# Ren91/gelly-streaming

Hardware: AMD Instinct MI355X
Metric: edges/sec per tumbling slice (reduceOnEdges, window triangles) at 1/2/4/8 GPUs (higher is better)
Workload: dtype int64

## Files before the change

gelly-streaming_amd/csrc/gs_bucket.hip:

```cpp
#include <algorithm>

#include "gs_ops.hpp"
#include <atomic>
#include <chrono>
#ifndef GS_DOM_ACCUM
#define GS_DOM_ACCUM 1
#endif

#include "gs_bucket.hpp"

namespace gs {

#ifndef GS_BK_ITEM_LOG
#define GS_BK_ITEM_LOG 17
#endif
#ifndef GS_BK_UNROLL
#define GS_BK_UNROLL 8
#endif
constexpr uint32_t BK_ITEM = 1u << GS_BK_ITEM_LOG;

namespace {

constexpr gs_status GS_RETRY_WIDE = -100;

struct BkMeta {
  static constexpr size_t HIST = 0, DBASE = HIST + BK_MAXB, BSTART = DBASE + 512, BCOUNT = BSTART + BK_MAXB + 4,
                          BITEMS = BCOUNT + BK_MAXB, BSLAB = BITEMS + BK_MAXB, MLIST = BSLAB + BK_MAXB,
                          MAXIT = MLIST + BK_MAXB,
                          TOTAL = MAXIT + 4;
};

struct BkGeom {
  int64_t base = 0;
  uint32_t nb = 1;
  int passes = 0, w = 0;
};

int64_t key_min(const uint64_t* h) { return (int64_t)(~h[0] ^ (1ull << 63)); }
int64_t key_max(const uint64_t* h) { return (int64_t)(h[1] ^ (1ull << 63)); }

int64_t predict_base(int64_t kmin, int64_t kmax, int S) {
  return (kmin >= 0 && ((uint64_t)kmax >> S) < (uint64_t)BK_MAXB) ? 0 : kmin;
}

template <int DIR>
// ... 74 lines not shown
uint32_t item_records(gs_ctx* c, uint64_t R) {
  const uint64_t per = R / (GS_BK_ITEMS_PER_CU * (uint64_t)std::max(1, c->n_cu));
  return (uint32_t)std::max<uint64_t>(BK_ITEM, std::min<uint64_t>(per, 1u << 20));
}

gs_status ensure_cu(gs_ctx* c) {
  if (!c->n_cu) {
    int cu = 0;
    GS_HIP(hipDeviceGetAttribute(&cu, hipDeviceAttributeMultiprocessorCount, c->device));
    c->n_cu = std::max(1, cu);
  }
  return GS_OK;
}

template <class P>
gs_status launch_plan(gs_ctx* c, uint64_t R, uint32_t nb, int passes, int w, uint32_t item_recs,
                      const uint32_t* cursor = nullptr, uint32_t* counts_out = nullptr,
                      unsigned long long* occupied = nullptr) {
  char* sm = c->small.as<char>();
  uint32_t* meta = c->bk_meta.as<uint32_t>();
  const uint64_t max_items = R / item_recs + nb + 1;
  const uint64_t max_slabs = 2 * (R / item_recs) + 2;
  GS_TRY(ensure(c, c->bk_items, max_items * sizeof(BkItem)));
  GS_TRY(ensure(c, c->bk_slabs, max_slabs * sizeof(typename P::Lds)));
  uint32_t* ns = (uint32_t*)(sm + SM_BK_N);
  BkPlanOut po{meta + BkMeta::DBASE, meta + BkMeta::BSTART, meta + BkMeta::BCOUNT, meta + BkMeta::BITEMS,
               meta + BkMeta::BSLAB, meta + BkMeta::MLIST, c->bk_items.as<BkItem>(), ns + 0, ns + 1,
               cursor, counts_out, occupied, ns + 2, meta + BkMeta::MAXIT};
  hipLaunchKernelGGL(k_bk_plan, dim3(1), dim3(BK_PLAN_BLOCK), 0, c->stream, meta + BkMeta::HIST, nb, passes, w,
                     item_recs, po);
  return hip_check(c, hipGetLastError(), "k_bk_plan");
}

template <class P, class Src>
gs_status bucket_accumulate(gs_ctx* c, Src rs, uint64_t R, uint32_t nb, int64_t base, typename P::Out o, int ev0,
                           const uint32_t* seg_cur = nullptr) {
  char* sm = c->small.as<char>();
  uint32_t* meta = c->bk_meta.as<uint32_t>();
  uint32_t* ns = (uint32_t*)(sm + SM_BK_N);
  const auto* mm = (const unsigned long long*)(sm + SM_BK_MM);
  BkStage st{c->keysA.as<uint32_t>(), c->valsA.p,
             (std::is_same_v<P, BkDeg> || std::is_same_v<P, BkDeg32>) ? c->aux.as<int64_t>() : nullptr};
  auto* slabs = c->bk_slabs.as<typename P::Lds>();
  const bool dom = GS_DOM_ACCUM && ev0 == 2 && c->timing == GS_TIMING_DOMINANT;
  launch_dominant(c, dom ? c->pass_ev[7] : nullptr, dom ? c->pass_ev[ev0 + 1] : nullptr, k_bk_accum<P, Src, GS_BK_UNROLL>,
                  dim3(c->n_cu * GS_BK_ACC_PER_CU), dim3(BK_ACC_BLOCK), rs, (const BkItem*)c->bk_items.as<BkItem>(),
                  (const uint32_t*)(ns + 0), (const uint32_t*)(meta + BkMeta::BSTART), ns + 2, slabs, st,
                  meta + BkMeta::BCOUNT, mm, seg_cur);
  GS_HIP(hipGetLastError());
  stage_event(c, c->pass_ev[ev0 + 1]);
  const unsigned mgrid = (unsigned)std::max<uint64_t>(1, std::min<uint64_t>({(uint64_t)nb, R / BK_ITEM + 1, 64}));
  const unsigned fgrid = (unsigned)std::max<uint64_t>(1, std::min<uint64_t>({(uint64_t)nb, R / BK_ITEM + 1, (uint64_t)c->n_cu}));
  hipLaunchKernelGGL((k_bk_merge_groups<P>), dim3(2048), dim3(BK_MS_BLOCK), 0, c->stream, meta + BkMeta::MLIST, ns + 1,
                     meta + BkMeta::BITEMS, meta + BkMeta::BSLAB, slabs, mm, (const uint32_t*)(meta + BkMeta::MAXIT));
  hipLaunchKernelGGL((k_bk_merge_slices<P>), dim3(mgrid, BK_MS_SLICES), dim3(BK_MS_BLOCK), 0, c->stream,
                     meta + BkMeta::MLIST, ns + 1, meta + BkMeta::BITEMS, meta + BkMeta::BSLAB, slabs, mm);
  hipLaunchKernelGGL((k_bk_merge<P>), dim3(fgrid), dim3(BK_ACC_BLOCK), 0, c->stream, meta + BkMeta::MLIST, ns + 1,
                     meta + BkMeta::BITEMS, meta + BkMeta::BSLAB, meta + BkMeta::BSTART, slabs, st,
                     meta + BkMeta::BCOUNT, mm);
  GS_HIP(hipGetLastError());
  stage_event(c, c->pass_ev[ev0 + 2]);
  if (c->oe.nparts) {
    const OwnerEmit& e = c->oe;
    hipLaunchKernelGGL(k_bk_owner_count, dim3(nb, BK_OE_SLICES), dim3(256), 0, c->stream, (const uint32_t*)(meta + BkMeta::BSTART),
                       (const uint32_t*)(meta + BkMeta::BCOUNT), nb, (const uint32_t*)st.k, base, e.nparts, e.cnt, e.wide,
                       mm, (const uint32_t*)(sm + SM_TIMEOUT), (const unsigned long long*)(sm + SM_BK_ESC),
                       (unsigned long long*)(sm + SM_BK_X));
    hipLaunchKernelGGL(k_owner_scan, dim3(1), dim3(1024), 0, c->stream, e.cnt, nb * BK_OE_SLICES * e.nparts,
                       nb * BK_OE_SLICES, e.nparts, e.totals,
                       (unsigned long long*)(sm + SM_BK_MM + 24));
    hipLaunchKernelGGL((k_bk_owner_emit<P>), dim3(nb, BK_OE_SLICES), dim3(256), 0, c->stream, (const uint32_t*)(meta + BkMeta::BSTART),
                       (const uint32_t*)(meta + BkMeta::BCOUNT), nb, st, base, o, e.nparts, (const uint32_t*)e.cnt, e.rows,
                       (const unsigned long long*)e.wide, e.vw, e.mw, mm);
    hipLaunchKernelGGL(k_send_rows, dim3(1), dim3(64), 0, c->stream, (const unsigned long long*)e.totals, e.wide,
// ... 169 lines not shown
        SpSlots slots{};
        const uint32_t xmask = c->sp_slot == 0 ? 7u : 0u;
        if (!xmask) {
          for (uint32_t x = 1; x <= SP_NSEG; ++x) slots.pre[x] = (uint32_t)R;
        } else {
          const uint64_t tr = (DIR == DIR_ALL ? 2 : 1) * SPTE, nfull = n / SPTE, per = (nfull + 7) / 8;
          uint64_t acc = 0;
          for (uint32_t x = 0; x < SP_NSEG; ++x) {
            slots.pre[x] = (uint32_t)acc;
            const uint64_t lo = std::min<uint64_t>(nfull, SP_NSEG == 1 ? 0 : x * per);
            const uint64_t hi = SP_NSEG == 1 ? nfull : std::min<uint64_t>(nfull, (x + 1) * per);
            acc += (hi - lo) * tr + (x == 0 ? R - nfull * tr : 0);
          }
          slots.pre[SP_NSEG] = (uint32_t)acc;
        }
        hipLaunchKernelGGL(k_sp_regions, dim3(1), dim3(BK_PLAN_BLOCK), 0, c->stream, (const uint32_t*)sp.tot.as<uint32_t>(),
                           nb, sp.R, R, meta + BkMeta::BSTART, c->sp_cur.as<uint32_t>(), slots, mm,
                           (unsigned long long*)(sm + SM_BK_ESC));
        if constexpr (P::REL) GS_HIP(hipMemsetAsync(rel_bad, 0, 4, c->stream));
        stage_event(c, c->ev[1]);
        stage_event(c, c->pass_ev[0]);
        stage_event(c, c->pass_ev[1]);
        using Load = typename P::Load;
        const BaseSrc<Load, DIR, P::PAY> ls{src, dst, (const Load*)val, base};
        uint32_t* cur = c->sp_cur.as<uint32_t>();
        hipEvent_t e0 = c->pass_ev[1], e1 = c->pass_ev[2];
        uint32_t* kp = c->keysB.as<uint32_t>();
        auto* esc = (unsigned long long*)(sm + SM_BK_ESC);
        const uint32_t trash = (uint32_t)cap;
        if constexpr (CAN_PACK && ITEMS == PK_ITEMS) {
          if (pack && nb <= 1024)
            launch_dominant(c, e0, e1, k_sp_scatter_pack<Load, DIR, 1024>, dim3(spk_grid<DIR>(n)), dim3(SPK_BLOCK), ls, n,
                            S, nb, cur, kp, vpart, trash, mm, esc, xmask);
// ... 2 lines not shown
                            n, S, nb, cur, kp, vpart, trash, mm, esc, xmask);
        }
        if constexpr (ITEMS == DP_ITEMS) {
          if (!pack) {
            if (nb <= 1024)
              launch_dominant(c, e0, e1, k_sp_scatter<Load, DIR, P::PAY, Raw, P::REL, 1024>, dim3(spu_grid<DIR>(n)),
                              dim3(SPU_BLOCK), ls, n, S, nb, cur, k16, vpart, trash, rel_bad, mm, xmask);
            else
              launch_dominant(c, e0, e1, k_sp_scatter<Load, DIR, P::PAY, Raw, P::REL, BK_MAXB>, dim3(spu_grid<DIR>(n)),
                              dim3(SPU_BLOCK), ls, n, S, nb, cur, k16, vpart, trash, rel_bad, mm, xmask);
          }
        }
        GS_HIP(hipGetLastError());
        stage_event(c, c->pass_ev[2]);
        stage_event(c, c->ev[2]);
        GS_TRY(launch_plan<P>(c, cap, nb, 0, 0, item_recs, cur, sp.tot.as<uint32_t>(), mm));
        part = true;
        if (pack) GS_TRY((bucket_accumulate<P>(c, PackSrc<Raw>{c->keysB.as<uint32_t>(), vpart}, cap, nb, base, o, 2, cur)));
        else GS_TRY((bucket_accumulate<P>(c, PartSrc<Raw>{k16, vpart}, cap, nb, base, o, 2, cur)));
        if (defer) return GS_PENDING_LOCAL;
        GS_TRY(bucket_wait(c));
        if (!c->host_small[2]) {
          kmin = (int64_t)((uint64_t)base + (c->host_small[0] << S));
          kmax = (int64_t)((uint64_t)base + (c->host_small[1] << S) + ((1ull << S) - 1));
          break;
        }
        sp.skip = 8;
        spec = false;
        spec_missed = true;
        continue;
      }
    }
    GS_TRY((launch_dp_hist<DIR, ITEMS>(c, src, dst, n, nt, base, S, nb)));
    GS_HIP(hipMemsetAsync(sm + SM_BK_ESC, 0, 8, c->stream));
// ... 76 lines not shown
  const uint64_t esc = pack ? c->host_small[7] : 0;
  const uint32_t key_bits = nb <= 1 ? (uint32_t)S : (uint32_t)(S + 32 - __builtin_clz(nb - 1));
  const size_t pb = pack ? 2 : (P::HAS_V ? sizeof(Raw) : 0);
  bucket_times(c, 2, part ? 1 : 0, 5, key_bits, R, *U, pb, n_items);
  c->times.key_bytes = 2;
  c->times.escapes = esc;
  c->times.packed = pack ? 1u : 0u;
  c->times.speculative = spec ? 1u : spec_missed ? 2u : 0u;
  if constexpr (SPEC_OK) {
    if (part) {
      sp.ok = true;
      sp.base = base;
      sp.S = S;
      sp.dir = DIR;
      sp.R = R;
    }
  }
  return GS_OK;
}

template <class P, int DIR>
gs_status bucket_direct(gs_ctx* c, const int64_t* src, const int64_t* dst, const void* val, uint64_t n,
                        typename P::Out o, uint64_t* U) {
  constexpr bool CAN_PACK = P::PAY == PAY_VAL && !P::REL && std::is_integral_v<typename P::A>;
  if constexpr (CAN_PACK) {
    if (c->bk_wide_vals[c->sp_slot] <= 0 && !(c->flags & GS_FLAG_NO_PACK))
      return bucket_direct_t<P, DIR, PK_ITEMS>(c, src, dst, val, n, o, U, true);
  }
  return bucket_direct_t<P, DIR, DP_ITEMS>(c, src, dst, val, n, o, U, false);
}
// ... 144 lines not shown
```

gelly-streaming_amd/csrc/gs_bucket.hpp:

```cpp
#pragma once
#include <limits>
#include <type_traits>

#include "gs_radix.hpp"
#include "gs_rbk.hpp"

namespace gs {

constexpr int BK_MAXB = 2048;
constexpr int BK_INFO_BLOCK = 512;
#ifndef GS_BK_ACC_BLOCK
#define GS_BK_ACC_BLOCK 1024
#endif
#ifndef GS_BK_ACC_PER_CU
#define GS_BK_ACC_PER_CU 1
#endif
#ifndef GS_BK_PREFETCH
#define GS_BK_PREFETCH 0
#endif
#ifndef GS_BK_FUSED_RESET
#define GS_BK_FUSED_RESET 1
#endif
#ifndef GS_BK_S8
#define GS_BK_S8 14
#endif
constexpr int BK_ACC_BLOCK = GS_BK_ACC_BLOCK;
constexpr int BK_NW = BK_ACC_BLOCK / WAVE;
constexpr int BK_PLAN_BLOCK = 1024;

struct BkItem {
  uint32_t bucket, begin, end, slab;
};

struct BkStage {
  uint32_t* k;
  void* a;
  int64_t* b;
};

struct BkPlanOut {
  uint32_t* digit_base;
  uint32_t* bucket_start;
  uint32_t* bucket_count;
  uint32_t* b_items;
  uint32_t* b_slab;
  uint32_t* mlist;
  BkItem* items;
  uint32_t* n_items;
  uint32_t* n_multi;
  const uint32_t* cursor = nullptr;
  uint32_t* counts_out = nullptr;
  unsigned long long* occupied = nullptr;
  uint32_t* claim = nullptr;
  uint32_t* max_items = nullptr;
};

#ifndef GS_SP_XCD
#define GS_SP_XCD 1
#endif
constexpr uint32_t SP_NSEG = GS_SP_XCD ? 8 : 1;
#ifndef GS_SP_MATCH
#define GS_SP_MATCH 1
#endif
constexpr uint32_t SP_PAD = 1024;
constexpr uint32_t SP_PADSEG = SP_PAD / SP_NSEG;
static_assert(SP_PADSEG % 4 == 0, "segment starts stay 4-aligned");
constexpr uint32_t SP_END_OFF = SP_NSEG * BK_MAXB;
constexpr uint32_t SP_LO_OFF = 2 * SP_NSEG * BK_MAXB;
constexpr uint32_t SP_CUR_WORDS = 3 * SP_NSEG * BK_MAXB;
// ... 419 lines not shown
#pragma unroll
  for (int i = 0; i < NW; ++i) {
    const uint32_t v = s_w[i];
    off += i < w ? v : 0u;
    tot += v;
  }
  __syncthreads();
  total = tot;
  return off + inc - x;
}

#ifndef GS_BK_LPT
#define GS_BK_LPT 1
#endif
constexpr int BK_LPT_CLASSES = 64;
static __global__ __launch_bounds__(BK_PLAN_BLOCK) void k_bk_plan(const uint32_t* __restrict__ hist, uint32_t nb,
                                                                  int passes, int w, uint32_t item_recs,
                                                                  BkPlanOut o) {
  __shared__ uint32_t s_dh[2][256];
  __shared__ uint32_t s_w[BK_PLAN_BLOCK / WAVE];
  __shared__ uint32_t s_maxit;
  const int tid = threadIdx.x;
  for (int i = tid; i < 2 * 256; i += BK_PLAN_BLOCK) (&s_dh[0][0])[i] = 0;
  if (tid == 0) s_maxit = 0;
  if (tid == 0 && o.claim) *o.claim = 0;
  __syncthreads();
  const uint32_t b0 = 2 * tid, b1 = 2 * tid + 1;
  const bool spec = o.cursor != nullptr;
  auto count = [&](uint32_t b) -> uint32_t {
    if (b >= nb) return 0u;
    if (!spec) return hist[b];
    uint32_t n = 0;
    for (uint32_t x = 0; x < SP_NSEG; ++x) n += min(o.cursor[x * BK_MAXB + b], sp_hi(o.cursor, x, b)) - sp_lo(o.cursor, x, b);
    return n;
  };
  const uint32_t c0 = count(b0), c1 = count(b1);
  const uint32_t dmask = (1u << w) - 1;
  for (int p = 0; p < passes; ++p) {
    if (c0) atomicAdd(&s_dh[p][(b0 >> (p * w)) & dmask], c0);
// ... 22 lines not shown
    o.counts_out[b0] = c0;
    o.counts_out[b1] = c1;
  }
  if (!spec) {
    if (b0 < nb) o.bucket_start[b0] = start0;
    if (b1 < nb) o.bucket_start[b1] = start0 + c0;
    if (tid == 0) o.bucket_start[nb] = total;
  }
  if (tid < passes) {
    uint32_t run = 0;
    for (uint32_t d = 0; d <= dmask; ++d) {
      o.digit_base[tid * 256 + d] = run;
      run += s_dh[tid][d];
    }
  }
  auto nitems = [&](uint32_t c) { return c == 0 ? 0u : (c + item_recs - 1) / item_recs; };
  const uint32_t i0 = nitems(c0), i1 = nitems(c1);
  const uint32_t m0 = i0 > 1 ? i0 : 0u, m1 = i1 > 1 ? i1 : 0u;
  uint32_t n_items, n_slabs, n_multi;
  const uint32_t first0 = bk_block_scan(i0 + i1, s_w, n_items);
  const uint32_t slab0 = bk_block_scan(m0 + m1, s_w, n_slabs);
  const uint32_t mb0 = bk_block_scan((m0 ? 1u : 0u) + (m1 ? 1u : 0u), s_w, n_multi);
#if GS_BK_LPT
  __shared__ uint32_t s_cls[BK_LPT_CLASSES];
  for (int i = tid; i < BK_LPT_CLASSES; i += BK_PLAN_BLOCK) s_cls[i] = 0;
  __syncthreads();
  auto size_class = [&](uint32_t n) -> uint32_t {
    return BK_LPT_CLASSES - 1 - min<uint32_t>(BK_LPT_CLASSES - 1, (uint32_t)((uint64_t)n * BK_LPT_CLASSES / (item_recs + 1)));
  };
  auto count_items = [&](uint32_t b, uint32_t c, uint32_t ni) {
    if (b >= nb || !ni) return;
    if (ni > 1) atomicAdd(&s_cls[size_class(item_recs)], ni - 1);
    atomicAdd(&s_cls[size_class(c - (ni - 1) * item_recs)], 1u);
  };
  count_items(b0, c0, i0);
  count_items(b1, c1, i1);
  __syncthreads();
  static_assert(BK_LPT_CLASSES == WAVE, "one wave scans the classes");
  if (tid < WAVE) {
    const uint32_t x = s_cls[tid];
    s_cls[tid] = wave_inclusive_sum(x) - x;
  }
  __syncthreads();
#endif
  auto emit_bucket = [&](uint32_t b, uint32_t c, uint32_t ni, uint32_t first, uint32_t slab, uint32_t mb) {
    if (b >= nb) return;
    o.bucket_count[b] = 0;
    o.b_items[b] = ni;
    o.b_slab[b] = slab;
    if (ni > 1) o.mlist[mb] = b;
    if (!ni) return;
#if GS_BK_LPT
    const uint32_t fpos = ni > 1 ? atomicAdd(&s_cls[size_class(item_recs)], ni - 1) : 0u;
    const uint32_t lpos = atomicAdd(&s_cls[size_class(c - (ni - 1) * item_recs)], 1u);
#endif
    for (uint32_t k = 0; k < ni; ++k) {
      BkItem it;
      it.bucket = b;
      it.begin = k * item_recs;
      it.end = min(c, (k + 1) * item_recs);
      it.slab = ni > 1 ? slab + k : ~0u;
#if GS_BK_LPT
      o.items[k + 1 < ni ? fpos + k : lpos] = it;
#else
      o.items[first + k] = it;
#endif
    }
  };
  emit_bucket(b0, c0, i0, first0, slab0, mb0);
  emit_bucket(b1, c1, i1, first0 + i0, slab0 + m0, mb0 + (m0 ? 1u : 0u));
  if (o.max_items) {
    if (i0 > 1 || i1 > 1) atomicMax(&s_maxit, max(i0, i1));
    __syncthreads();
  }
  if (tid == 0) {
    if (o.max_items) *o.max_items = s_maxit;
    *o.n_items = n_items;
    *o.n_multi = n_multi;
  }
}

#ifndef GS_DP_ITEMS
#define GS_DP_ITEMS 10
#endif
#ifndef GS_DP_XCD
#define GS_DP_XCD 1
#endif
#ifndef GS_DP_VDIRECT
#define GS_DP_VDIRECT 0
#endif
constexpr int DP_BLOCK = 1024;
constexpr int DP_ITEMS = GS_DP_ITEMS;
constexpr uint32_t DP_TILE = DP_BLOCK * DP_ITEMS;
constexpr uint32_t DP_CHUNK = 64;
// ... 383 lines not shown
    for (int u = 0; u < ITEMS; ++u) put((uint32_t)u * DP_BLOCK + tid);
  } else {
    for (uint32_t j = tid; j < nrec; j += DP_BLOCK) put(j);
  }
#pragma unroll
  for (int o = 32; o > 0; o >>= 1) esc += __shfl_xor(esc, o, WAVE);
  if ((tid & 63) == 0 && esc) atomicAdd(n_esc, (unsigned long long)esc);
}


static __global__ __launch_bounds__(BK_PLAN_BLOCK) void k_sp_regions(const uint32_t* __restrict__ prev, uint32_t nb,
                                                                     uint64_t r_prev, uint64_t r_now,
                                                                     uint32_t* __restrict__ bucket_start,
                                                                     uint32_t* __restrict__ cursor, SpSlots slots,
                                                                     unsigned long long* __restrict__ mm,
                                                                     unsigned long long* __restrict__ n_esc) {
  __shared__ uint32_t s_w[BK_PLAN_BLOCK / WAVE];
  __shared__ uint32_t s_frac[SP_NSEG + 1];
  const int tid = threadIdx.x;
  const uint32_t b0 = 2 * tid, b1 = 2 * tid + 1;
  if (tid <= (int)SP_NSEG) {
    const uint32_t all = slots.pre[SP_NSEG];
    const uint64_t f = all ? ((uint64_t)slots.pre[tid] << 32) / all : 0;
    s_frac[tid] = (uint32_t)min(f, (uint64_t)0xFFFFFFFFu);
  }
  auto cap = [&](uint32_t b) -> uint32_t {
    if (b >= nb) return 0u;
    const uint64_t t = (uint64_t)prev[b] * r_now / (r_prev ? r_prev : 1);
    return (uint32_t)((t + (t >> 4) + 3) & ~3ull) + SP_PAD;
  };
  const uint32_t c0 = cap(b0), c1 = cap(b1);
// ... 6 lines not shown
    const uint32_t h0 = sp_seg_start(s0, s0 + c0, x + 1, s_frac), h1 = sp_seg_start(s0 + c0, s0 + c0 + c1, x + 1, s_frac);
    if (b0 < nb) {
      cursor[x * BK_MAXB + b0] = l0;
      cursor[SP_LO_OFF + x * BK_MAXB + b0] = l0;
      cursor[SP_END_OFF + x * BK_MAXB + b0] = h0;
    }
    if (b1 < nb) {
      cursor[x * BK_MAXB + b1] = l1;
      cursor[SP_LO_OFF + x * BK_MAXB + b1] = l1;
      cursor[SP_END_OFF + x * BK_MAXB + b1] = h1;
    }
    l0 = h0;
    l1 = h1;
  }
  if (tid == 0) bucket_start[nb] = total;
  if (tid < 4) mm[tid] = 0;
  if (tid == 4) *n_esc = 0;
}

__host__ __device__ inline uint64_t sp_capacity(uint64_t r_now, uint32_t nb) {
  return r_now + (r_now >> 4) + (uint64_t)nb * (SP_PAD + 4);
}

#ifndef GS_SPK_BLOCK
#define GS_SPK_BLOCK 512
#endif
#ifndef GS_SPK_ITEMS
#define GS_SPK_ITEMS 16
#endif
#ifndef GS_SPK_NT
#define GS_SPK_NT 0
#endif
// ... 460 lines not shown
    const uint64_t m = ballot(p);
    if (p) {
      const uint32_t pos = stage_at + off + mbcnt(m);
      st.k[pos] = cbase | e;
      P::stage(st, pos, s, e);
    }
    off += (uint32_t)__popcll(m);
  }
  if constexpr (RESET) {
    static_assert(PER % 32 == 0, "a wave's entries are whole presence words");
    P::init_range(s, e0, e0 + PER, lane);
  }
  if (tid == 0) bucket_count[bucket] = tot;
}

#ifdef GS_BK_TRACE
constexpr uint32_t BK_TRACE_MAX = 16384;
__device__ uint64_t g_bk_trace[BK_TRACE_MAX][4];
#endif
template <class P, class Src, int UNROLL>
__global__ __launch_bounds__(BK_ACC_BLOCK) void k_bk_accum(Src src, const BkItem* __restrict__ items,
                                                           const uint32_t* __restrict__ n_items_p,
                                                           const uint32_t* __restrict__ bucket_start,
                                                           uint32_t* __restrict__ ctr,
                                                           typename P::Lds* __restrict__ slabs, BkStage st,
                                                           uint32_t* __restrict__ bucket_count,
                                                           const unsigned long long* __restrict__ mm,
                                                           const uint32_t* __restrict__ seg_cur) {
  __shared__ typename P::Lds s;
  __shared__ uint32_t s_item[2], s_b0[2];
  __shared__ BkItem s_m[2];
  __shared__ uint32_t s_wc[BK_NW];
  __shared__ uint32_t s_pre4[2][SP_NSEG + 1], s_qb[2][SP_NSEG];
  using Raw = typename P::Raw;
  constexpr bool PACKED = is_pack_src<Src>::value;
  const int tid = threadIdx.x, lane = tid & (WAVE - 1);
  if (mm[2]) return;
  const uint32_t n_items = *n_items_p;
  auto add1 = [&](const auto& sr, uint32_t q, uint32_t x) {
    const uint32_t v16 = x >> 16;
    const bool esc = v16 == PK_ESC;
    if constexpr (has_add_packed<P>::value) P::add_packed(s, x & (P::W - 1), !esc ? (Raw)v16 : (Raw)sr.wide[q], esc);
    else P::add(s, x & (P::W - 1), !esc ? (Raw)v16 : (Raw)sr.wide[q]);
  };
  uint32_t hq = 0, hx = 0;
  bool hh = false;
  auto prepare = [&](int b) {
    uint32_t it = 0;
    if (lane == 0) it = atomicAdd(ctr, 1u);
    it = __shfl(it, 0, WAVE);
    if (lane == 0) s_item[b] = it;
    hh = false;
    if (it >= n_items) return;
    const BkItem m = items[it];
    const uint32_t b0 = bucket_start[m.bucket];
    if (lane == 0) {
      s_m[b] = m;
      s_b0[b] = b0;
    }
    if constexpr (PACKED) {
      if (seg_cur) {
        const bool on = lane < (int)SP_NSEG;
        const uint32_t x = on ? (uint32_t)lane : 0u;
        const uint32_t sg = sp_lo(seg_cur, x, m.bucket);
        const uint32_t nx = on ? min(seg_cur[x * BK_MAXB + m.bucket], sp_hi(seg_cur, x, m.bucket)) - sg : 0u;
        const uint32_t at = wave_inclusive_sum(nx) - nx;
        const uint32_t lo = max(m.begin, at), hi = min(m.end, at + nx);
        uint32_t p0 = 0, p1 = 0;
        if (on && lo < hi) {
          p0 = sg + (lo - at);
          p1 = sg + (hi - at);
        }
        const uint32_t a0 = min(p1, (p0 + 3) & ~3u), a1 = max(a0, p1 & ~3u);
        const uint32_t n4 = (a1 - a0) / 4;
        const uint32_t e4 = wave_inclusive_sum(n4);
        if (on) {
          s_pre4[b][x + 1] = e4;
          s_qb[b][x] = a0 / 4 - (e4 - n4);
        }
        if (lane == 0) s_pre4[b][0] = 0;
        const uint32_t px = (uint32_t)lane / 6, j = (uint32_t)lane % 6;
        const uint32_t xp0 = __shfl(p0, (int)px, WAVE), xa0 = __shfl(a0, (int)px, WAVE);
        const uint32_t xa1 = __shfl(a1, (int)px, WAVE), xp1 = __shfl(p1, (int)px, WAVE);
        const uint32_t q = j < 3 ? xp0 + j : xa1 + (j - 3);
        hh = px < SP_NSEG && (j < 3 ? q < xa0 : q < xp1);
        if (hh) {
          hq = q;
          hx = src.rec[q];
        }
      }
    }
  };
  if (tid < WAVE) prepare(0);
  P::init(s, tid);
  __syncthreads();
  constexpr int U4 = UNROLL / 2 > 0 ? UNROLL / 2 : 1;
  uint4 xp[U4];
  uint32_t qp[U4];
  bool pf = false;
  for (int sl = 0;; sl ^= 1) {
    const uint32_t it = s_item[sl];
    if (it >= n_items) break;
    const BkItem m = s_m[sl];
    const uint32_t b0 = s_b0[sl];
#ifdef GS_BK_TRACE
// ... 165 lines not shown
        const uint4* rec4 = reinterpret_cast<const uint4*>(src.rec);
#pragma unroll
        for (int u = 0; u < U4; ++u) {
          const uint32_t g0 = (uint32_t)tid + (uint32_t)u * BK_ACC_BLOCK, g = g0 < n4n ? g0 : n4n - 1;
          uint32_t b = dq[0];
#pragma unroll
          for (uint32_t x = 1; x < SP_NSEG; ++x) b += g >= pre[x] ? dq[x] : 0u;
          qp[u] = g + b;
          xp[u] = rec4[qp[u]];
        }
        pf = true;
      }
    }
#endif
    bool reset = false;
    if (m.slab == ~0u) {
      bk_finalize<P, GS_BK_FUSED_RESET != 0>(s, m.bucket, b0, st, bucket_count, s_wc);
      reset = GS_BK_FUSED_RESET != 0;
    } else {
      const uint4* ls = reinterpret_cast<const uint4*>(&s);
      uint4* gs = reinterpret_cast<uint4*>(slabs + m.slab);
      for (uint32_t i = tid; i < sizeof(typename P::Lds) / 16; i += BK_ACC_BLOCK) gs[i] = ls[i];
    }
    __syncthreads();
#ifdef GS_BK_TRACE
    if (tid == 0 && it < BK_TRACE_MAX) {
      g_bk_trace[it][0] = blockIdx.x;
      g_bk_trace[it][1] = t_item0;
      g_bk_trace[it][2] = wall_clock64();
      g_bk_trace[it][3] = m.end - m.begin;
    }
#endif
    if (!reset) {
      P::init(s, tid);
      __syncthreads();
    }
  }
// ... 264 lines not shown
```

gelly-streaming_amd/csrc/gs_internal.hpp:

```cpp
#pragma once
#include <hip/hip_runtime.h>
#include <hip/hip_ext.h>
#include <stdint.h>

#include <string>

#include "../../include/gelly_hip.h"

namespace gs {

struct DevBuf {
  void* p = nullptr;
  size_t bytes = 0;
  template <typename T>
  T* as() const { return static_cast<T*>(p); }
};

struct OwnerEmit {
  uint32_t nparts = 0;
  uint32_t* rows = nullptr;
  uint32_t* cnt = nullptr;
  unsigned long long* totals = nullptr;
  unsigned long long* wide = nullptr;
  int vw = 0, mw = 0;
// ... 64 lines not shown
  gs::RtSplit rt_split{};
  uint64_t rt_n = ~0ull, rt_seq = 0;
  uint32_t rt_nparts = 0;
  gs::DevBuf tri_bd[4];
  gs::DevBuf tri_rl[4];
  gs::DevBuf hs[40];
  gs::DevBuf hs_rank;
  gs::DevBuf bk_meta, bk_items, bk_slabs;
  gs::DevBuf dp_cnt, dp_csum, dp_off;
  struct SpState {
    gs::DevBuf tot;
    bool ok = false;
    int S = 0, dir = -1, skip = 0;
    int64_t base = 0;
    uint64_t R = 0;
  } sp[2];
  int sp_slot = 0;
  uint64_t tri_merge = 0;
  gs::OwnerEmit oe;
  gs::DevBuf sp_cur;
  gs::DevBuf pr_a, pr_b, pr_f, pr_key, pr_val, pr_gk, pr_gv, pr_small;
  gs::DevBuf tx_text, tx_cnt, tx_starts;
  gs::DevBuf dist_k, dist_v, dist_v2, dist_k2, dist_v3, dist_v4, dist_cnt, dist_x, dist_x2;
  void* comm = nullptr;
  int comm_kind = 0;
  int comm_size = 0, comm_rank = 0;
  gs::DevBuf comm_scratch;
  gs::DevBuf rl[8];
  gs::DevBuf zipf_cdf;
  uint64_t zipf_v = 0;
// ... 119 lines not shown
```

Before: 186.9 billion.

## Merge small multi-item buckets inline in accumulate and plan early

Buckets split into at most a small number of items (GS_BK_INLINE_K) are now merged by the last-arriving accumulate block, which counts arrivals with an atomic counter per bucket. That block folds the sibling slabs and finalizes the bucket itself, so the separate merge kernels can be skipped when no larger buckets exist. The plan is also moved into the spill-regions kernel so the standalone plan launch is dropped, and bucket counts and the min/max bucket are written from accumulate. The cost is added atomics, fences and cross-block ordering complexity in the hot accumulate kernel.

```diff
diff --git a/gelly-streaming_amd/csrc/gs_bucket.hip b/gelly-streaming_amd/csrc/gs_bucket.hip
--- a/gelly-streaming_amd/csrc/gs_bucket.hip
+++ b/gelly-streaming_amd/csrc/gs_bucket.hip
@@ -17,18 +17,14 @@
 #ifndef GS_BK_UNROLL
 #define GS_BK_UNROLL 8
 #endif
+#ifndef GS_BK_PLAN_EARLY
+#define GS_BK_PLAN_EARLY 1
+#endif
 constexpr uint32_t BK_ITEM = 1u << GS_BK_ITEM_LOG;
 
 namespace {
 
 constexpr gs_status GS_RETRY_WIDE = -100;
-
-struct BkMeta {
-  static constexpr size_t HIST = 0, DBASE = HIST + BK_MAXB, BSTART = DBASE + 512, BCOUNT = BSTART + BK_MAXB + 4,
-                          BITEMS = BCOUNT + BK_MAXB, BSLAB = BITEMS + BK_MAXB, MLIST = BSLAB + BK_MAXB,
-                          MAXIT = MLIST + BK_MAXB,
-                          TOTAL = MAXIT + 4;
-};
 
 struct BkGeom {
   int64_t base = 0;
@@ -133,9 +129,8 @@
 }
 
 template <class P>
-gs_status launch_plan(gs_ctx* c, uint64_t R, uint32_t nb, int passes, int w, uint32_t item_recs,
-                      const uint32_t* cursor = nullptr, uint32_t* counts_out = nullptr,
-                      unsigned long long* occupied = nullptr) {
+gs_status plan_out(gs_ctx* c, uint64_t R, uint32_t nb, uint32_t item_recs, const uint32_t* cursor, uint32_t* counts_out,
+                   unsigned long long* occupied, BkPlanOut* po) {
   char* sm = c->small.as<char>();
   uint32_t* meta = c->bk_meta.as<uint32_t>();
   const uint64_t max_items = R / item_recs + nb + 1;
@@ -143,17 +138,27 @@
   GS_TRY(ensure(c, c->bk_items, max_items * sizeof(BkItem)));
   GS_TRY(ensure(c, c->bk_slabs, max_slabs * sizeof(typename P::Lds)));
   uint32_t* ns = (uint32_t*)(sm + SM_BK_N);
-  BkPlanOut po{meta + BkMeta::DBASE, meta + BkMeta::BSTART, meta + BkMeta::BCOUNT, meta + BkMeta::BITEMS,
-               meta + BkMeta::BSLAB, meta + BkMeta::MLIST, c->bk_items.as<BkItem>(), ns + 0, ns + 1,
-               cursor, counts_out, occupied, ns + 2, meta + BkMeta::MAXIT};
+  *po = BkPlanOut{meta + BkMeta::DBASE, meta + BkMeta::BSTART, meta + BkMeta::BCOUNT, meta + BkMeta::BITEMS,
+                  meta + BkMeta::BSLAB, meta + BkMeta::MLIST, c->bk_items.as<BkItem>(), ns + 0, ns + 1,
+                  cursor, counts_out, occupied, ns + 2, meta + BkMeta::MAXIT, meta + BkMeta::ARRIVE};
+  return GS_OK;
+}
+
+template <class P>
+gs_status launch_plan(gs_ctx* c, uint64_t R, uint32_t nb, int passes, int w, uint32_t item_recs,
+                      const uint32_t* cursor = nullptr, uint32_t* counts_out = nullptr,
+                      unsigned long long* occupied = nullptr, bool expect_no_merge = false) {
+  uint32_t* meta = c->bk_meta.as<uint32_t>();
+  BkPlanOut po;
+  GS_TRY(plan_out<P>(c, R, nb, item_recs, cursor, counts_out, occupied, &po));
   hipLaunchKernelGGL(k_bk_plan, dim3(1), dim3(BK_PLAN_BLOCK), 0, c->stream, meta + BkMeta::HIST, nb, passes, w,
-                     item_recs, po);
+                     item_recs, bk_inline_k<P>(), expect_no_merge && occupied, po);
   return hip_check(c, hipGetLastError(), "k_bk_plan");
 }
 
 template <class P, class Src>
 gs_status bucket_accumulate(gs_ctx* c, Src rs, uint64_t R, uint32_t nb, int64_t base, typename P::Out o, int ev0,
-                           const uint32_t* seg_cur = nullptr) {
+                           const uint32_t* seg_cur = nullptr, bool skip_merge = false, uint32_t* counts_out = nullptr) {
   char* sm = c->small.as<char>();
   uint32_t* meta = c->bk_meta.as<uint32_t>();
   uint32_t* ns = (uint32_t*)(sm + SM_BK_N);
@@ -164,19 +169,21 @@
   const bool dom = GS_DOM_ACCUM && ev0 == 2 && c->timing == GS_TIMING_DOMINANT;
   launch_dominant(c, dom ? c->pass_ev[7] : nullptr, dom ? c->pass_ev[ev0 + 1] : nullptr, k_bk_accum<P, Src, GS_BK_UNROLL>,
                   dim3(c->n_cu * GS_BK_ACC_PER_CU), dim3(BK_ACC_BLOCK), rs, (const BkItem*)c->bk_items.as<BkItem>(),
-                  (const uint32_t*)(ns + 0), (const uint32_t*)(meta + BkMeta::BSTART), ns + 2, slabs, st,
-                  meta + BkMeta::BCOUNT, mm, seg_cur);
+                  (const uint32_t*)(meta + BkMeta::BSTART), slabs, st, meta + BkMeta::BCOUNT,
+                  (unsigned long long*)(sm + SM_BK_MM), seg_cur, counts_out);
   GS_HIP(hipGetLastError());
   stage_event(c, c->pass_ev[ev0 + 1]);
   const unsigned mgrid = (unsigned)std::max<uint64_t>(1, std::min<uint64_t>({(uint64_t)nb, R / BK_ITEM + 1, 64}));
   const unsigned fgrid = (unsigned)std::max<uint64_t>(1, std::min<uint64_t>({(uint64_t)nb, R / BK_ITEM + 1, (uint64_t)c->n_cu}));
-  hipLaunchKernelGGL((k_bk_merge_groups<P>), dim3(2048), dim3(BK_MS_BLOCK), 0, c->stream, meta + BkMeta::MLIST, ns + 1,
-                     meta + BkMeta::BITEMS, meta + BkMeta::BSLAB, slabs, mm, (const uint32_t*)(meta + BkMeta::MAXIT));
-  hipLaunchKernelGGL((k_bk_merge_slices<P>), dim3(mgrid, BK_MS_SLICES), dim3(BK_MS_BLOCK), 0, c->stream,
-                     meta + BkMeta::MLIST, ns + 1, meta + BkMeta::BITEMS, meta + BkMeta::BSLAB, slabs, mm);
-  hipLaunchKernelGGL((k_bk_merge<P>), dim3(fgrid), dim3(BK_ACC_BLOCK), 0, c->stream, meta + BkMeta::MLIST, ns + 1,
-                     meta + BkMeta::BITEMS, meta + BkMeta::BSLAB, meta + BkMeta::BSTART, slabs, st,
-                     meta + BkMeta::BCOUNT, mm);
+  if (!skip_merge) {
+    hipLaunchKernelGGL((k_bk_merge_groups<P>), dim3(2048), dim3(BK_MS_BLOCK), 0, c->stream, meta + BkMeta::MLIST, ns + 1,
+                       meta + BkMeta::BITEMS, meta + BkMeta::BSLAB, slabs, mm, (const uint32_t*)(meta + BkMeta::MAXIT));
+    hipLaunchKernelGGL((k_bk_merge_slices<P>), dim3(mgrid, BK_MS_SLICES), dim3(BK_MS_BLOCK), 0, c->stream,
+                       meta + BkMeta::MLIST, ns + 1, meta + BkMeta::BITEMS, meta + BkMeta::BSLAB, slabs, mm);
+    hipLaunchKernelGGL((k_bk_merge<P>), dim3(fgrid), dim3(BK_ACC_BLOCK), 0, c->stream, meta + BkMeta::MLIST, ns + 1,
+                       meta + BkMeta::BITEMS, meta + BkMeta::BSLAB, meta + BkMeta::BSTART, slabs, st,
+                       meta + BkMeta::BCOUNT, mm);
+  }
   GS_HIP(hipGetLastError());
   stage_event(c, c->pass_ev[ev0 + 2]);
   if (c->oe.nparts) {
@@ -376,9 +383,13 @@
           }
           slots.pre[SP_NSEG] = (uint32_t)acc;
         }
+        const bool no_merge = bk_inline_k<P>() > 1 && sp.n_merge == 0;
+        constexpr bool PLAN_EARLY = GS_BK_PLAN_EARLY && bk_inline_k<P>() > 1;
+        BkPlanOut po{};
+        if (PLAN_EARLY) GS_TRY(plan_out<P>(c, cap, nb, item_recs, nullptr, nullptr, nullptr, &po));
         hipLaunchKernelGGL(k_sp_regions, dim3(1), dim3(BK_PLAN_BLOCK), 0, c->stream, (const uint32_t*)sp.tot.as<uint32_t>(),
                            nb, sp.R, R, meta + BkMeta::BSTART, c->sp_cur.as<uint32_t>(), slots, mm,
-                           (unsigned long long*)(sm + SM_BK_ESC));
+                           (unsigned long long*)(sm + SM_BK_ESC), item_recs, bk_inline_k<P>(), no_merge, po);
         if constexpr (P::REL) GS_HIP(hipMemsetAsync(rel_bad, 0, 4, c->stream));
         stage_event(c, c->ev[1]);
         stage_event(c, c->pass_ev[0]);
@@ -411,10 +422,13 @@
         GS_HIP(hipGetLastError());
         stage_event(c, c->pass_ev[2]);
         stage_event(c, c->ev[2]);
-        GS_TRY(launch_plan<P>(c, cap, nb, 0, 0, item_recs, cur, sp.tot.as<uint32_t>(), mm));
+        if (!PLAN_EARLY) GS_TRY(launch_plan<P>(c, cap, nb, 0, 0, item_recs, cur, sp.tot.as<uint32_t>(), mm, no_merge));
         part = true;
-        if (pack) GS_TRY((bucket_accumulate<P>(c, PackSrc<Raw>{c->keysB.as<uint32_t>(), vpart}, cap, nb, base, o, 2, cur)));
-        else GS_TRY((bucket_accumulate<P>(c, PartSrc<Raw>{k16, vpart}, cap, nb, base, o, 2, cur)));
+        uint32_t* counts = PLAN_EARLY ? sp.tot.as<uint32_t>() : nullptr;
+        if (pack)
+          GS_TRY((bucket_accumulate<P>(c, PackSrc<Raw>{c->keysB.as<uint32_t>(), vpart}, cap, nb, base, o, 2, cur, no_merge,
+                                       counts)));
+        else GS_TRY((bucket_accumulate<P>(c, PartSrc<Raw>{k16, vpart}, cap, nb, base, o, 2, cur, no_merge, counts)));
         if (defer) return GS_PENDING_LOCAL;
         GS_TRY(bucket_wait(c));
         if (!c->host_small[2]) {
@@ -521,6 +535,7 @@
       sp.S = S;
       sp.dir = DIR;
       sp.R = R;
+      sp.n_merge = std::max<uint32_t>((uint32_t)(c->host_small[4] >> 32), spec ? 0u : 1u);
     }
   }
   return GS_OK;
diff --git a/gelly-streaming_amd/csrc/gs_bucket.hpp b/gelly-streaming_amd/csrc/gs_bucket.hpp
--- a/gelly-streaming_amd/csrc/gs_bucket.hpp
+++ b/gelly-streaming_amd/csrc/gs_bucket.hpp
@@ -2,6 +2,7 @@
 #include <limits>
 #include <type_traits>
 
+#include "gs_internal.hpp"
 #include "gs_radix.hpp"
 #include "gs_rbk.hpp"
 
@@ -18,6 +19,13 @@
 #ifndef GS_BK_PREFETCH
 #define GS_BK_PREFETCH 0
 #endif
+#ifndef GS_BK_INLINE_K
+#define GS_BK_INLINE_K 4
+#endif
+template <class P>
+__host__ __device__ constexpr uint32_t bk_inline_k() {
+  return std::is_integral_v<typename P::A> && GS_BK_INLINE_K > 1 ? (uint32_t)GS_BK_INLINE_K : 0u;
+}
 #ifndef GS_BK_FUSED_RESET
 #define GS_BK_FUSED_RESET 1
 #endif
@@ -36,6 +44,14 @@
   uint32_t* k;
   void* a;
   int64_t* b;
+};
+
+struct BkMeta {
+  static constexpr size_t HIST = 0, DBASE = HIST + BK_MAXB, BSTART = DBASE + 512, BCOUNT = BSTART + BK_MAXB + 4,
+                          BITEMS = BCOUNT + BK_MAXB, BSLAB = BITEMS + BK_MAXB, MLIST = BSLAB + BK_MAXB,
+                          MAXIT = MLIST + BK_MAXB,
+                          ARRIVE = MAXIT + 4,
+                          TOTAL = ARRIVE + BK_MAXB;
 };
 
 struct BkPlanOut {
@@ -53,6 +69,7 @@
   unsigned long long* occupied = nullptr;
   uint32_t* claim = nullptr;
   uint32_t* max_items = nullptr;
+  uint32_t* arrive = nullptr;
 };
 
 #ifndef GS_SP_XCD
@@ -502,15 +519,92 @@
 #define GS_BK_LPT 1
 #endif
 constexpr int BK_LPT_CLASSES = 64;
+__device__ __forceinline__ uint32_t bk_plan_items(uint32_t c0, uint32_t c1, uint32_t nb, uint32_t item_recs,
+                                                  uint32_t inline_k, const BkPlanOut& o, uint32_t* s_w) {
+  __shared__ uint32_t s_maxit;
+  const int tid = threadIdx.x;
+  const uint32_t b0 = 2 * tid, b1 = 2 * tid + 1;
+  if (tid == 0) s_maxit = 0;
+  auto nitems = [&](uint32_t c) { return c == 0 ? 0u : (c + item_recs - 1) / item_recs; };
+  const uint32_t i0 = nitems(c0), i1 = nitems(c1);
+  const uint32_t m0 = i0 > 1 ? i0 : 0u, m1 = i1 > 1 ? i1 : 0u;
+  const uint32_t lk = max(1u, inline_k);
+  const uint32_t g0 = i0 > lk ? 1u : 0u, g1 = i1 > lk ? 1u : 0u;
+  uint32_t n_items, n_slabs, n_multi;
+  const uint32_t first0 = bk_block_scan(i0 + i1, s_w, n_items);
+  const uint32_t slab0 = bk_block_scan(m0 + m1, s_w, n_slabs);
+  const uint32_t mb0 = bk_block_scan(g0 + g1, s_w, n_multi);
+#if GS_BK_LPT
+  __shared__ uint32_t s_cls[BK_LPT_CLASSES];
+  for (int i = tid; i < BK_LPT_CLASSES; i += BK_PLAN_BLOCK) s_cls[i] = 0;
+  __syncthreads();
+  auto size_class = [&](uint32_t n) -> uint32_t {
+    return BK_LPT_CLASSES - 1 - min<uint32_t>(BK_LPT_CLASSES - 1, (uint32_t)((uint64_t)n * BK_LPT_CLASSES / (item_recs + 1)));
+  };
+  auto count_items = [&](uint32_t b, uint32_t c, uint32_t ni) {
+    if (b >= nb || !ni) return;
+    const bool together = ni > 1 && ni <= inline_k;
+    if (ni > 1) atomicAdd(&s_cls[size_class(item_recs)], together ? ni : ni - 1);
+    if (!together) atomicAdd(&s_cls[size_class(c - (ni - 1) * item_recs)], 1u);
+  };
+  count_items(b0, c0, i0);
+  count_items(b1, c1, i1);
+  __syncthreads();
+  static_assert(BK_LPT_CLASSES == WAVE, "one wave scans the classes");
+  if (tid < WAVE) {
+    const uint32_t x = s_cls[tid];
+    s_cls[tid] = wave_inclusive_sum(x) - x;
+  }
+  __syncthreads();
+#endif
+  auto emit_bucket = [&](uint32_t b, uint32_t c, uint32_t ni, uint32_t first, uint32_t slab, uint32_t mb) {
+    if (b >= nb) return;
+    o.bucket_count[b] = 0;
+    o.b_items[b] = ni;
+    o.b_slab[b] = slab;
+    if (o.arrive) o.arrive[b] = 0;
+    if (ni > lk) o.mlist[mb] = b;
+    if (!ni) return;
+#if GS_BK_LPT
+    const bool together = ni > 1 && ni <= inline_k;
+    const uint32_t fpos = ni > 1 ? atomicAdd(&s_cls[size_class(item_recs)], together ? ni : ni - 1) : 0u;
+    const uint32_t lpos = together ? fpos + ni - 1 : atomicAdd(&s_cls[size_class(c - (ni - 1) * item_recs)], 1u);
+#endif
+    for (uint32_t k = 0; k < ni; ++k) {
+      BkItem it;
+      it.bucket = b;
+      it.begin = k * item_recs;
+      it.end = min(c, (k + 1) * item_recs);
+      it.slab = ni > 1 ? slab + k : ~0u;
+#if GS_BK_LPT
+      o.items[k + 1 < ni ? fpos + k : lpos] = it;
+#else
+      o.items[first + k] = it;
+#endif
+    }
+  };
+  emit_bucket(b0, c0, i0, first0, slab0, mb0);
+  emit_bucket(b1, c1, i1, first0 + i0, slab0 + m0, mb0 + g0);
+  if (o.max_items) {
+    if (i0 > 1 || i1 > 1) atomicMax(&s_maxit, max(i0, i1));
+    __syncthreads();
+  }
+  if (tid == 0) {
+    if (o.max_items) *o.max_items = s_maxit;
+    *o.n_items = n_items;
+    *o.n_multi = n_multi;
+  }
+  return n_multi;
+}
+
 static __global__ __launch_bounds__(BK_PLAN_BLOCK) void k_bk_plan(const uint32_t* __restrict__ hist, uint32_t nb,
                                                                   int passes, int w, uint32_t item_recs,
+                                                                  uint32_t inline_k, bool expect_no_merge,
                                                                   BkPlanOut o) {
   __shared__ uint32_t s_dh[2][256];
   __shared__ uint32_t s_w[BK_PLAN_BLOCK / WAVE];
-  __shared__ uint32_t s_maxit;
   const int tid = threadIdx.x;
   for (int i = tid; i < 2 * 256; i += BK_PLAN_BLOCK) (&s_dh[0][0])[i] = 0;
-  if (tid == 0) s_maxit = 0;
   if (tid == 0 && o.claim) *o.claim = 0;
   __syncthreads();
   const uint32_t b0 = 2 * tid, b1 = 2 * tid + 1;
@@ -563,70 +657,8 @@
       run += s_dh[tid][d];
     }
   }
-  auto nitems = [&](uint32_t c) { return c == 0 ? 0u : (c + item_recs - 1) / item_recs; };
-  const uint32_t i0 = nitems(c0), i1 = nitems(c1);
-  const uint32_t m0 = i0 > 1 ? i0 : 0u, m1 = i1 > 1 ? i1 : 0u;
-  uint32_t n_items, n_slabs, n_multi;
-  const uint32_t first0 = bk_block_scan(i0 + i1, s_w, n_items);
-  const uint32_t slab0 = bk_block_scan(m0 + m1, s_w, n_slabs);
-  const uint32_t mb0 = bk_block_scan((m0 ? 1u : 0u) + (m1 ? 1u : 0u), s_w, n_multi);
-#if GS_BK_LPT
-  __shared__ uint32_t s_cls[BK_LPT_CLASSES];
-  for (int i = tid; i < BK_LPT_CLASSES; i += BK_PLAN_BLOCK) s_cls[i] = 0;
-  __syncthreads();
-  auto size_class = [&](uint32_t n) -> uint32_t {
-    return BK_LPT_CLASSES - 1 - min<uint32_t>(BK_LPT_CLASSES - 1, (uint32_t)((uint64_t)n * BK_LPT_CLASSES / (item_recs + 1)));
-  };
-  auto count_items = [&](uint32_t b, uint32_t c, uint32_t ni) {
-    if (b >= nb || !ni) return;
-    if (ni > 1) atomicAdd(&s_cls[size_class(item_recs)], ni - 1);
-    atomicAdd(&s_cls[size_class(c - (ni - 1) * item_recs)], 1u);
-  };
-  count_items(b0, c0, i0);
-  count_items(b1, c1, i1);
-  __syncthreads();
-  static_assert(BK_LPT_CLASSES == WAVE, "one wave scans the classes");
-  if (tid < WAVE) {
-    const uint32_t x = s_cls[tid];
-    s_cls[tid] = wave_inclusive_sum(x) - x;
-  }
-  __syncthreads();
-#endif
-  auto emit_bucket = [&](uint32_t b, uint32_t c, uint32_t ni, uint32_t first, uint32_t slab, uint32_t mb) {
-    if (b >= nb) return;
-    o.bucket_count[b] = 0;
-    o.b_items[b] = ni;
-    o.b_slab[b] = slab;
-    if (ni > 1) o.mlist[mb] = b;
-    if (!ni) return;
-#if GS_BK_LPT
-    const uint32_t fpos = ni > 1 ? atomicAdd(&s_cls[size_class(item_recs)], ni - 1) : 0u;
-    const uint32_t lpos = atomicAdd(&s_cls[size_class(c - (ni - 1) * item_recs)], 1u);
-#endif
-    for (uint32_t k = 0; k < ni; ++k) {
-      BkItem it;
-      it.bucket = b;
-      it.begin = k * item_recs;
-      it.end = min(c, (k + 1) * item_recs);
-      it.slab = ni > 1 ? slab + k : ~0u;
-#if GS_BK_LPT
-      o.items[k + 1 < ni ? fpos + k : lpos] = it;
-#else
-      o.items[first + k] = it;
-#endif
-    }
-  };
-  emit_bucket(b0, c0, i0, first0, slab0, mb0);
-  emit_bucket(b1, c1, i1, first0 + i0, slab0 + m0, mb0 + (m0 ? 1u : 0u));
-  if (o.max_items) {
-    if (i0 > 1 || i1 > 1) atomicMax(&s_maxit, max(i0, i1));
-    __syncthreads();
-  }
-  if (tid == 0) {
-    if (o.max_items) *o.max_items = s_maxit;
-    *o.n_items = n_items;
-    *o.n_multi = n_multi;
-  }
+  const uint32_t n_multi = bk_plan_items(c0, c1, nb, item_recs, inline_k, o, s_w);
+  if (tid == 0 && expect_no_merge && n_multi) atomicAdd(&o.occupied[2], 1ull);
 }
 
 #ifndef GS_DP_ITEMS
@@ -1040,7 +1072,9 @@
                                                                      uint32_t* __restrict__ bucket_start,
                                                                      uint32_t* __restrict__ cursor, SpSlots slots,
                                                                      unsigned long long* __restrict__ mm,
-                                                                     unsigned long long* __restrict__ n_esc) {
+                                                                     unsigned long long* __restrict__ n_esc,
+                                                                     uint32_t item_recs, uint32_t inline_k,
+                                                                     bool expect_no_merge, BkPlanOut plan) {
   __shared__ uint32_t s_w[BK_PLAN_BLOCK / WAVE];
   __shared__ uint32_t s_frac[SP_NSEG + 1];
   const int tid = threadIdx.x;
@@ -1077,8 +1111,19 @@
     l1 = h1;
   }
   if (tid == 0) bucket_start[nb] = total;
-  if (tid < 4) mm[tid] = 0;
   if (tid == 4) *n_esc = 0;
+  if (!plan.items) {
+    if (tid < 4) mm[tid] = 0;
+    return;
+  }
+  if (tid == 0) *plan.claim = 0;
+  const uint32_t n_multi = bk_plan_items(c0, c1, nb, item_recs, inline_k, plan, s_w);
+  if (tid == 0) {
+    mm[0] = ~0u;
+    mm[1] = 0;
+    mm[2] = expect_no_merge && n_multi ? 1 : 0;
+    mm[3] = 0;
+  }
 }
 
 __host__ __device__ inline uint64_t sp_capacity(uint64_t r_now, uint32_t nb) {
@@ -1569,21 +1614,47 @@
   if (tid == 0) bucket_count[bucket] = tot;
 }
 
+template <class P>
+__device__ __attribute__((noinline)) void bk_merge_slabs(typename P::Lds* s, const typename P::Lds* first, uint32_t ni,
+                                                         uint32_t mine, uint32_t empties) {
+  const uint32_t tid = threadIdx.x;
+  for (uint32_t k = 0; k < ni; ++k) {
+    if (k == mine || ((empties >> k) & 1u)) continue;
+    const typename P::Lds* g = first + k;
+#pragma unroll 4
+    for (uint32_t i = tid; i < P::W; i += BK_ACC_BLOCK) P::merge_el(s, g, i);
+    for (uint32_t w = tid; w < P::PWORDS; w += BK_ACC_BLOCK) P::merge_pw(s, g, w);
+  }
+}
+
 #ifdef GS_BK_TRACE
 constexpr uint32_t BK_TRACE_MAX = 16384;
 __device__ uint64_t g_bk_trace[BK_TRACE_MAX][4];
 #endif
 template <class P, class Src, int UNROLL>
 __global__ __launch_bounds__(BK_ACC_BLOCK) void k_bk_accum(Src src, const BkItem* __restrict__ items,
-                                                           const uint32_t* __restrict__ n_items_p,
                                                            const uint32_t* __restrict__ bucket_start,
-                                                           uint32_t* __restrict__ ctr,
                                                            typename P::Lds* __restrict__ slabs, BkStage st,
                                                            uint32_t* __restrict__ bucket_count,
-                                                           const unsigned long long* __restrict__ mm,
-                                                           const uint32_t* __restrict__ seg_cur) {
+                                                           unsigned long long* __restrict__ mm,
+                                                           const uint32_t* __restrict__ seg_cur,
+                                                           uint32_t* __restrict__ counts_out) {
+  static_assert(SM_BK_N == SM_BK_MM + 4 * sizeof(unsigned long long), "ns = mm + 4");
+  static_assert(BkMeta::BCOUNT < BkMeta::BITEMS && BkMeta::BITEMS < BkMeta::BSLAB && BkMeta::BSLAB < BkMeta::ARRIVE &&
+                    BkMeta::ARRIVE + BK_MAXB <= BkMeta::TOTAL,
+                "b_items, b_slab and the arrival counters follow bucket_count inside bk_meta");
+  uint32_t* const ns = reinterpret_cast<uint32_t*>(mm + 4);
+  uint32_t* const ctr = ns + 2;
+  const uint32_t* const b_items = bucket_count + (BkMeta::BITEMS - BkMeta::BCOUNT);
+  const uint32_t* const b_slab = bucket_count + (BkMeta::BSLAB - BkMeta::BCOUNT);
+  uint32_t* const arrive = bucket_count + (BkMeta::ARRIVE - BkMeta::BCOUNT);
   __shared__ typename P::Lds s;
   __shared__ uint32_t s_item[2], s_b0[2];
+  __shared__ uint32_t s_ni[2], s_f[2];
+  __shared__ uint32_t s_last;
+  __shared__ uint32_t s_nrec[2], s_tot[2];
+  constexpr uint32_t IK = bk_inline_k<P>();
+  static_assert(IK <= 16, "the arrival counter: 8 bits of tickets, a bit per empty item above them");
   __shared__ BkItem s_m[2];
   __shared__ uint32_t s_wc[BK_NW];
   __shared__ uint32_t s_pre4[2][SP_NSEG + 1], s_qb[2][SP_NSEG];
@@ -1591,7 +1662,7 @@
   constexpr bool PACKED = is_pack_src<Src>::value;
   const int tid = threadIdx.x, lane = tid & (WAVE - 1);
   if (mm[2]) return;
-  const uint32_t n_items = *n_items_p;
+  const uint32_t n_items = ns[0];
   auto add1 = [&](const auto& sr, uint32_t q, uint32_t x) {
     const uint32_t v16 = x >> 16;
     const bool esc = v16 == PK_ESC;
@@ -1613,14 +1684,35 @@
       s_m[b] = m;
       s_b0[b] = b0;
     }
-    if constexpr (PACKED) {
-      if (seg_cur) {
-        const bool on = lane < (int)SP_NSEG;
-        const uint32_t x = on ? (uint32_t)lane : 0u;
-        const uint32_t sg = sp_lo(seg_cur, x, m.bucket);
-        const uint32_t nx = on ? min(seg_cur[x * BK_MAXB + m.bucket], sp_hi(seg_cur, x, m.bucket)) - sg : 0u;
-        const uint32_t at = wave_inclusive_sum(nx) - nx;
-        const uint32_t lo = max(m.begin, at), hi = min(m.end, at + nx);
+    if constexpr (IK > 1) {
+      if (m.slab != ~0u) {
+        const uint32_t ni = b_items[m.bucket], f = b_slab[m.bucket];
+        if (lane == 0) {
+          s_ni[b] = ni;
+          s_f[b] = f;
+        }
+      }
+    }
+    uint32_t nrec = m.end - m.begin, tot = 1;
+    if (seg_cur && (PACKED || counts_out)) {
+      const bool on = lane < (int)SP_NSEG;
+      const uint32_t x = on ? (uint32_t)lane : 0u;
+      const uint32_t sg = sp_lo(seg_cur, x, m.bucket);
+      const uint32_t nx = on ? min(seg_cur[x * BK_MAXB + m.bucket], sp_hi(seg_cur, x, m.bucket)) - sg : 0u;
+      const uint32_t inc = wave_inclusive_sum(nx), at = inc - nx;
+      const uint32_t lo = max(m.begin, at), hi = min(m.end, at + nx);
+      if (counts_out) {
+        tot = __shfl(inc, WAVE - 1, WAVE);
+        nrec = __shfl(wave_inclusive_sum(on && lo < hi ? hi - lo : 0u), WAVE - 1, WAVE);
+        if (lane == 0 && m.begin == 0) {
+          counts_out[m.bucket] = tot;
+          if (tot) {
+            atomicMin(&mm[0], (unsigned long long)m.bucket);
+            atomicMax(&mm[1], (unsigned long long)m.bucket);
+          }
+        }
+      }
+      if constexpr (PACKED) {
         uint32_t p0 = 0, p1 = 0;
         if (on && lo < hi) {
           p0 = sg + (lo - at);
@@ -1644,6 +1736,10 @@
           hx = src.rec[q];
         }
       }
+    }
+    if (lane == 0) {
+      s_nrec[b] = nrec;
+      s_tot[b] = tot;
     }
   };
   if (tid < WAVE) prepare(0);
@@ -1839,13 +1935,69 @@
     }
 #endif
     bool reset = false;
+    const uint32_t nrec = s_nrec[sl];
     if (m.slab == ~0u) {
-      bk_finalize<P, GS_BK_FUSED_RESET != 0>(s, m.bucket, b0, st, bucket_count, s_wc);
-      reset = GS_BK_FUSED_RESET != 0;
+      if (nrec) bk_finalize<P, GS_BK_FUSED_RESET != 0>(s, m.bucket, b0, st, bucket_count, s_wc);
+      reset = !nrec || GS_BK_FUSED_RESET != 0;
     } else {
-      const uint4* ls = reinterpret_cast<const uint4*>(&s);
-      uint4* gs = reinterpret_cast<uint4*>(slabs + m.slab);
-      for (uint32_t i = tid; i < sizeof(typename P::Lds) / 16; i += BK_ACC_BLOCK) gs[i] = ls[i];
+      bool last = false, merged = false, idle = false;
+      uint32_t ni = 0, f = 0, mine = 0, empties = 0;
+      auto arrived = [&](uint32_t v) { return (v & 0xFFu) == ni - 1 ? 0x80000000u | (v >> 8) : 0u; };
+      if constexpr (IK > 1) {
+        ni = s_ni[sl];
+        f = s_f[sl];
+        mine = m.slab - f;
+        merged = ni <= IK && s_tot[sl] != 0;
+        if (merged) {
+          if (tid == 0)
+            s_last = arrived(__hip_atomic_load(&arrive[m.bucket], __ATOMIC_RELAXED, __HIP_MEMORY_SCOPE_AGENT));
+          __syncthreads();
+          last = s_last != 0;
+          empties = s_last & 0xFFFFu;
+        }
+        idle = ni <= IK && !nrec;
+        if (idle) reset = true;
+      }
+      if (!last && !idle) {
+        const uint4* ls = reinterpret_cast<const uint4*>(&s);
+        uint4* gs = reinterpret_cast<uint4*>(slabs + m.slab);
+        for (uint32_t i = tid; i < sizeof(typename P::Lds) / 16; i += BK_ACC_BLOCK) gs[i] = ls[i];
+        if constexpr (IK > 1) {
+          if (merged) {
+            asm volatile("s_waitcnt vmcnt(0)" ::: "memory");
+            __syncthreads();
+            if (tid == 0) {
+              __builtin_amdgcn_fence(__ATOMIC_RELEASE, "agent");
+              asm volatile("s_waitcnt vmcnt(0)" ::: "memory");
+              s_last = arrived(__hip_atomic_fetch_add(&arrive[m.bucket], 1u, __ATOMIC_RELAXED, __HIP_MEMORY_SCOPE_AGENT));
+            }
+            __syncthreads();
+            last = s_last != 0;
+            empties = s_last & 0xFFFFu;
+          }
+        }
+      } else if (!last && merged) {
+        __syncthreads();
+        if (tid == 0)
+          s_last = arrived(__hip_atomic_fetch_add(&arrive[m.bucket], 1u | (0x100u << mine), __ATOMIC_RELAXED,
+                                                  __HIP_MEMORY_SCOPE_AGENT));
+        __syncthreads();
+        last = s_last != 0;
+        empties = s_last & 0xFFFFu;
+      }
+      if constexpr (IK > 1) {
+        if (last) {
+          if (tid == 0) {
+            __builtin_amdgcn_fence(__ATOMIC_ACQUIRE, "agent");
+            asm volatile("s_waitcnt vmcnt(0)" ::: "memory");
+          }
+          __syncthreads();
+          bk_merge_slabs<P>(&s, slabs + f, ni, mine, empties);
+          __syncthreads();
+          bk_finalize<P, GS_BK_FUSED_RESET != 0>(s, m.bucket, b0, st, bucket_count, s_wc);
+          reset = GS_BK_FUSED_RESET != 0;
+        }
+      }
     }
     __syncthreads();
 #ifdef GS_BK_TRACE
diff --git a/gelly-streaming_amd/csrc/gs_internal.hpp b/gelly-streaming_amd/csrc/gs_internal.hpp
--- a/gelly-streaming_amd/csrc/gs_internal.hpp
+++ b/gelly-streaming_amd/csrc/gs_internal.hpp
@@ -102,6 +102,7 @@
     int S = 0, dir = -1, skip = 0;
     int64_t base = 0;
     uint64_t R = 0;
+    uint32_t n_merge = 0;
   } sp[2];
   int sp_slot = 0;
   uint64_t tri_merge = 0;
```

After: 190.8 billion (median of 6 runs). 1.02x the previous value.
